# SysCV/LiDAR_snow_sim

Hardware: NVIDIA H100
Metric: augmented LiDAR points/sec (higher is better)
Workload: dtype f64

## Files before the change

include/lidar_snow_sim.h:

```cpp
#ifndef LIDAR_SNOW_SIM_H
#define LIDAR_SNOW_SIM_H

#include <stdint.h>

#ifdef __cplusplus
extern "C" {
#endif

#if defined(__GNUC__)
#define LSS_API __attribute__((visibility("default")))
#else
#define LSS_API
#endif

typedef struct lss_engine lss_engine;

typedef enum {
    LSS_OK = 0,
    LSS_ERR_INVALID_ARG = 1,
    LSS_ERR_CUDA = 2,
    LSS_ERR_NO_TABLE = 3,
    LSS_ERR_RANGE_INDEX = 4,
    LSS_ERR_NEGATIVE_INTENSITY = 5,
    LSS_ERR_OCCLUDER_OVERFLOW = 6,
    LSS_ERR_WORKSPACE = 7,
    LSS_ERR_NO_SENSOR = 8,
    LSS_ERR_TOO_FEW_GROUND = 9
} lss_status;

#define LSS_FLAG_THRESHOLD_FILTER 0x1u
#define LSS_FLAG_CAMERA_FOV 0x2u
#define LSS_FLAG_DEVICE_PREPASS 0x4u
#define LSS_FLAG_ASSUME_SORTED 0x8u

#define LSS_N_CHANNELS 64
#define LSS_POINT_STRIDE 5

LSS_API lss_status lss_create(int device, lss_engine **out);
LSS_API void lss_destroy(lss_engine *e);
LSS_API const char *lss_status_string(lss_status s);
LSS_API const char *lss_last_error(const lss_engine *e);
LSS_API int lss_version(void);

LSS_API lss_status lss_set_sensor(lss_engine *e, int n_channels, const double *h_focal_distance, const double *h_focal_slope,
                          const double *h_min_intensity, const double *h_max_intensity);

LSS_API lss_status lss_set_camera(lss_engine *e, const float *h_P2, const float *h_R0, const float *h_V2C, int img_h,
                          int img_w);

LSS_API lss_status lss_upload_particles(lss_engine *e, int n_planes, const double *h_xyr, const int64_t *h_plane_offsets,
                                double max_beam_divergence_rad, int n_azimuth_buckets, void *stream,
                                int *table_id_out);
LSS_API lss_status lss_upload_particles_device(lss_engine *e, int n_planes, const double *d_xyr,
                                       const int64_t *h_plane_offsets, double max_beam_divergence_rad,
                                       int n_azimuth_buckets, void *stream, int *table_id_out);
LSS_API lss_status lss_free_particles(lss_engine *e, int table_id);
LSS_API lss_status lss_table_info(lss_engine *e, int table_id, int64_t *n_particles, int64_t *n_entries, int64_t *bytes);

LSS_API lss_status lss_snowfall_batch(lss_engine *e, int table_id, const float *d_points, const int64_t *h_cloud_offsets,
                              int n_clouds, const int32_t *h_order, double beam_divergence_deg, const float *d_theta,
                              const double *h_thresh_poly, const double *h_plane_in, const int32_t *h_ymins_in,
                              double noise_floor, uint32_t flags, float *d_out_points,
                              int32_t *d_out_counts, double *d_out_stats, float *d_out_full, int32_t *d_out_perm,
                              int32_t *d_out_nocc, void *d_workspace, int64_t workspace_bytes, void *stream);
LSS_API int64_t lss_snowfall_workspace_bytes(int64_t n_total, int n_clouds);
LSS_API lss_status lss_snowfall_batch_host(lss_engine *e, int table_id, const float *h_points,
                                           const int64_t *h_cloud_offsets, int n_clouds, const int32_t *h_order,
                                           double beam_divergence_deg, const double *h_thresh_poly, double noise_floor,
                                           uint32_t flags, int n_chunks, float *h_out_points, int32_t *h_out_counts,
                                           double *h_out_stats);
LSS_API lss_status lss_snowfall_batch_host_submit(lss_engine *e, int table_id, const float *h_points,
                                                  const int64_t *h_cloud_offsets, int n_clouds, const int32_t *h_order,
                                                  double beam_divergence_deg, const double *h_thresh_poly,
                                                  double noise_floor, uint32_t flags, int n_chunks, float *h_out_points,
                                                  int32_t *h_out_counts, double *h_out_stats, int *ticket_out);
LSS_API lss_status lss_snowfall_batch_host_wait(lss_engine *e, int ticket);
LSS_API int lss_host_pipe_trace(lss_engine *e, float *out, int cap_chunks);
LSS_API lss_status lss_check_async(lss_engine *e, void *stream);
LSS_API int64_t lss_launch_count(const lss_engine *e);
LSS_API lss_status lss_noise_threshold_poly(lss_engine *e, const float *d_points, const int64_t *h_cloud_offsets,
                                    int n_clouds, double noise_floor, const double *h_plane_in,
                                    const int32_t *h_ymins_in, double *d_poly_out, double *d_plane_out,
                                    double *d_fit_out, int32_t *d_ymins_out, void *d_workspace,
                                    int64_t workspace_bytes, void *stream);
LSS_API int64_t lss_prepass_workspace_bytes(int64_t n_total, int n_clouds);

LSS_API lss_status lss_wet_ground_batch(lss_engine *e, const float *d_points, const int64_t *h_cloud_offsets,
                                const int32_t *d_cloud_counts, int n_clouds, double water_height, double pavement_depth,
                                double noise_floor, double power_factor, int flat_earth, double delta, int replace,
                                const double *h_plane_in, const int32_t *h_ymins_in, float *d_out_points,
                                double *d_out_intensity64, int32_t *d_out_counts, int32_t *d_out_passthrough,
                                double *d_out_plane, void *d_workspace, int64_t workspace_bytes, void *stream);
LSS_API int64_t lss_wet_ground_workspace_bytes(int64_t n_total, int n_clouds);

#define LSS_FOG_HARD 0x1u
#define LSS_FOG_SOFT 0x2u
#define LSS_FOG_GAIN 0x4u
LSS_API lss_status lss_fog_batch(lss_engine *e, const float *d_points, int n_features, const int64_t *h_cloud_offsets,
                                 int n_clouds, double alpha, double beta, double beta_0, const double *d_lut,
                                 uint32_t flags, int noise, int noise_variant, const uint64_t *h_rng_state,
                                 const double *d_ext_noise, double *d_out, uint8_t *d_out_fog_mask, int32_t *d_out_rank,
                                 double *d_out_info, void *d_workspace, int64_t workspace_bytes, void *stream);
LSS_API int64_t lss_fog_workspace_bytes(int64_t n_total, int n_clouds);
LSS_API lss_status lss_fog_batch_params(lss_engine *e, const float *d_points, int n_features,
                                        const int64_t *h_cloud_offsets, int n_clouds, const double *h_alpha,
                                        const double *h_beta, const double *h_beta_0, const int32_t *h_table_index,
                                        const double *d_luts, int n_tables, uint32_t flags, int noise, int noise_variant,
                                        const uint64_t *h_rng_state, const double *d_ext_noise, double *d_out,
                                        uint8_t *d_out_fog_mask, int32_t *d_out_rank, double *d_out_info,
                                        void *d_workspace, int64_t workspace_bytes, void *stream);
LSS_API int64_t lss_fog_batch_params_workspace_bytes(int64_t n_total, int n_clouds);

typedef struct lss_fog_table_params {
    double alpha, tau_h, r_1, r_2, D, ROH_T, ROH_R, GAMMA_T, GAMMA_R;
    double c_a, p_0, beta;
    double r_range, r_0_max, granularity;
    int32_t n, linear_xsi, shift, reserved;
} lss_fog_table_params;
LSS_API lss_status lss_fog_integral_tables(lss_engine *e, const lss_fog_table_params *h_params, int n_tables,
                                           double *d_out, void *d_workspace, int64_t workspace_bytes, void *stream);
LSS_API int64_t lss_fog_integral_tables_workspace_bytes(int n, int n_tables);

LSS_API lss_status lss_lisa_batch(lss_engine *e, const double *d_points, int n_features, int64_t n_points, double rain_rate,
                                  int mode, double alpha, double r_min, double r_max, double beam_divergence,
                                  double min_diameter, double range_accuracy, int signal_last,
                                  const double *d_draw_table, int table_len, uint64_t seed, double *d_out, void *stream);

LSS_API lss_status lss_voxelize_batch(lss_engine *e, const float *d_points, int n_features, const int64_t *h_cloud_offsets,
                                      const int32_t *d_cloud_counts, int n_clouds, const float *h_point_cloud_range,
                                      const float *h_voxel_size, int max_points_per_voxel, int max_voxels,
                                      int mask_xy_range, float *d_out_voxels, int32_t *d_out_coords,
                                      int32_t *d_out_num_points, int32_t *d_out_n_voxels, void *d_workspace,
                                      int64_t workspace_bytes, void *stream);
LSS_API int64_t lss_voxelize_workspace_bytes(int64_t n_total, int n_clouds, int max_points_per_voxel, int max_voxels);

#define LSS_DROR_CUBE 0x1u
#define LSS_DROR_WORK_STATS 0x100u
LSS_API lss_status lss_dror_batch(lss_engine *e, const float *d_points, int n_features, const int64_t *h_cloud_offsets,
                                  const int32_t *d_cloud_counts, int n_clouds, double alpha_deg, double beta, int k_min,
                                  double sr_min, uint32_t flags, uint8_t *d_out_keep ,
                                  float *d_out_points , int32_t *d_out_counts, int32_t *d_out_n_snow,
                                  void *d_workspace, int64_t workspace_bytes, void *stream);
LSS_API int64_t lss_dror_workspace_bytes(int64_t n_total, int n_clouds);

LSS_API lss_status lss_gather_push(lss_engine *e, const float *d_points, const int32_t *d_counts,
                                   const int64_t *d_cloud_offsets, int n_clouds, int64_t n_rows, int world, int rank,
                                   float *const *h_peer_points, int32_t *const *h_peer_counts, float *d_mc_points,
                                   int32_t *d_mc_counts, int n_blocks, void *stream);

LSS_API lss_status lss_dart_throwing(double occupancy_ratio, double precipitation_rate, double R_0, int distribution,
                             uint64_t *pcg_state, double *h_xyr, int64_t capacity, int64_t *n_out);
LSS_API lss_status lss_dart_throwing_planes(int n_planes, double occupancy_ratio, double precipitation_rate, double R_0,
                                    int distribution, uint64_t *pcg_states, double *h_xyr,
                                    int64_t capacity_per_plane, int64_t *h_counts, int n_threads);

LSS_API lss_status lss_sample_particles(lss_engine *e, int n_planes, double occupancy_ratio, double precipitation_rate,
                                double R_0, int distribution, uint64_t seed, int64_t n_candidates, double *d_xyr_out,
                                int64_t capacity_per_plane, int32_t *d_counts, double *d_candidates_out,
                                void *d_workspace, int64_t workspace_bytes, void *stream);
LSS_API int64_t lss_sample_particles_workspace_bytes(int n_planes, int64_t n_candidates);

LSS_API lss_status lss_set_profiling(lss_engine *e, int enable);
LSS_API lss_status lss_kernel_times(lss_engine *e, int reset, double *h_ms, int64_t *h_calls, int n);
LSS_API const char *lss_kernel_name(int kernel);
LSS_API lss_status lss_debug_azimuth(lss_engine *e, const float *d_y, const float *d_x, int64_t n, float *d_out, void *stream);
LSS_API lss_status lss_debug_range_grid(double *h_out);

#ifdef __cplusplus
}
#endif
#endif
```

lidar_snow_sim_b200/_lib.py:

```python
import ctypes
import os

_HERE = os.path.dirname(os.path.abspath(__file__))
LIB_PATH = os.path.join(_HERE, 'liblss_b200.so')

LSS_OK = 0
LSS_ERR_INVALID_ARG = 1
LSS_ERR_CUDA = 2
LSS_ERR_NO_TABLE = 3
LSS_ERR_RANGE_INDEX = 4
LSS_ERR_NEGATIVE_INTENSITY = 5
LSS_ERR_OCCLUDER_OVERFLOW = 6
LSS_ERR_WORKSPACE = 7
LSS_ERR_NO_SENSOR = 8
LSS_ERR_TOO_FEW_GROUND = 9

FLAG_THRESHOLD_FILTER = 0x1
FLAG_CAMERA_FOV = 0x2
FLAG_DEVICE_PREPASS = 0x4
FLAG_ASSUME_SORTED = 0x8
FOG_HARD, FOG_SOFT, FOG_GAIN = 0x1, 0x2, 0x4
DROR_CUBE, DROR_WORK_STATS = 0x1, 0x100



class FogTableParams(ctypes.Structure):
    _fields_ = [(f, ctypes.c_double) for f in ('alpha', 'tau_h', 'r_1', 'r_2', 'D', 'ROH_T', 'ROH_R', 'GAMMA_T',
                                                'GAMMA_R', 'c_a', 'p_0', 'beta', 'r_range', 'r_0_max', 'granularity')]
    _fields_ += [(f, ctypes.c_int32) for f in ('n', 'linear_xsi', 'shift', 'reserved')]


_EXC = {
    LSS_ERR_INVALID_ARG: ValueError,
    LSS_ERR_CUDA: RuntimeError,
    LSS_ERR_NO_TABLE: FileNotFoundError,
    LSS_ERR_RANGE_INDEX: IndexError,
    LSS_ERR_NEGATIVE_INTENSITY: AssertionError,
    LSS_ERR_OCCLUDER_OVERFLOW: RuntimeError,
    LSS_ERR_WORKSPACE: RuntimeError,
    LSS_ERR_NO_SENSOR: AssertionError,
    LSS_ERR_TOO_FEW_GROUND: TypeError,
}

_c = ctypes
_P = ctypes.c_void_p
SIGNATURES = [
    ('lss_create', _c.c_int, [_c.c_int, _c.POINTER(_P)]),
    ('lss_destroy', None, [_P]),
    ('lss_status_string', _c.c_char_p, [_c.c_int]),
    ('lss_last_error', _c.c_char_p, [_P]),
    ('lss_version', _c.c_int, []),
    ('lss_set_sensor', _c.c_int, [_P, _c.c_int, _P, _P, _P, _P]),
    ('lss_set_camera', _c.c_int, [_P, _P, _P, _P, _c.c_int, _c.c_int]),
    ('lss_upload_particles', _c.c_int, [_P, _c.c_int, _P, _P, _c.c_double, _c.c_int, _P, _c.POINTER(_c.c_int)]),
    ('lss_upload_particles_device', _c.c_int, [_P, _c.c_int, _P, _P, _c.c_double, _c.c_int, _P,
                                               _c.POINTER(_c.c_int)]),
    ('lss_free_particles', _c.c_int, [_P, _c.c_int]),
    ('lss_table_info', _c.c_int, [_P, _c.c_int, _c.POINTER(_c.c_int64), _c.POINTER(_c.c_int64),
                                  _c.POINTER(_c.c_int64)]),
    ('lss_snowfall_batch', _c.c_int, [_P, _c.c_int, _P, _P, _c.c_int, _P, _c.c_double, _P, _P, _P, _P, _c.c_double,
                                      _c.c_uint32, _P, _P, _P, _P, _P, _P, _P, _c.c_int64, _P]),
    ('lss_snowfall_workspace_bytes', _c.c_int64, [_c.c_int64, _c.c_int]),
    ('lss_host_pipe_trace', _c.c_int, [_P, _P, _c.c_int]),
    ('lss_snowfall_batch_host', _c.c_int, [_P, _c.c_int, _P, _P, _c.c_int, _P, _c.c_double, _P, _c.c_double, _c.c_uint32,
                                           _c.c_int, _P, _P, _P]),
    ('lss_snowfall_batch_host_submit', _c.c_int, [_P, _c.c_int, _P, _P, _c.c_int, _P, _c.c_double, _P, _c.c_double,
                                                  _c.c_uint32, _c.c_int, _P, _P, _P, _c.POINTER(_c.c_int)]),
    ('lss_snowfall_batch_host_wait', _c.c_int, [_P, _c.c_int]),
    ('lss_check_async', _c.c_int, [_P, _P]),
    ('lss_launch_count', _c.c_int64, [_P]),
    ('lss_debug_range_grid', _c.c_int, [_P]),
    ('lss_debug_azimuth', _c.c_int, [_P, _P, _P, _c.c_int64, _P, _P]),
    ('lss_noise_threshold_poly', _c.c_int, [_P, _P, _P, _c.c_int, _c.c_double, _P, _P, _P, _P, _P, _P, _P, _c.c_int64,
                                            _P]),
    ('lss_prepass_workspace_bytes', _c.c_int64, [_c.c_int64, _c.c_int]),
    ('lss_wet_ground_batch', _c.c_int, [_P, _P, _P, _P, _c.c_int, _c.c_double, _c.c_double, _c.c_double, _c.c_double,
                                        _c.c_int, _c.c_double, _c.c_int, _P, _P, _P, _P, _P, _P, _P, _P, _c.c_int64, _P]),
    ('lss_wet_ground_workspace_bytes', _c.c_int64, [_c.c_int64, _c.c_int]),
    ('lss_fog_batch', _c.c_int, [_P, _P, _c.c_int, _P, _c.c_int, _c.c_double, _c.c_double, _c.c_double, _P, _c.c_uint32,
                                 _c.c_int, _c.c_int, _P, _P, _P, _P, _P, _P, _P, _c.c_int64, _P]),
    ('lss_fog_workspace_bytes', _c.c_int64, [_c.c_int64, _c.c_int]),
    ('lss_fog_batch_params', _c.c_int, [_P, _P, _c.c_int, _P, _c.c_int, _P, _P, _P, _P, _P, _c.c_int, _c.c_uint32,
                                        _c.c_int, _c.c_int, _P, _P, _P, _P, _P, _P, _P, _c.c_int64, _P]),
    ('lss_fog_batch_params_workspace_bytes', _c.c_int64, [_c.c_int64, _c.c_int]),
    ('lss_fog_integral_tables', _c.c_int, [_P, _P, _c.c_int, _P, _P, _c.c_int64, _P]),
    ('lss_fog_integral_tables_workspace_bytes', _c.c_int64, [_c.c_int, _c.c_int]),
    ('lss_lisa_batch', _c.c_int, [_P, _P, _c.c_int, _c.c_int64, _c.c_double, _c.c_int, _c.c_double, _c.c_double, _c.c_double,
                                  _c.c_double, _c.c_double, _c.c_double, _c.c_int, _P, _c.c_int, _c.c_uint64, _P, _P]),
    ('lss_voxelize_batch', _c.c_int, [_P, _P, _c.c_int, _P, _P, _c.c_int, _P, _P, _c.c_int, _c.c_int, _c.c_int, _P, _P, _P,
                                      _P, _P, _c.c_int64, _P]),
    ('lss_voxelize_workspace_bytes', _c.c_int64, [_c.c_int64, _c.c_int, _c.c_int, _c.c_int]),
    ('lss_dror_batch', _c.c_int, [_P, _P, _c.c_int, _P, _P, _c.c_int, _c.c_double, _c.c_double, _c.c_int, _c.c_double,
                                  _c.c_uint32, _P, _P, _P, _P, _P, _c.c_int64, _P]),
    ('lss_dror_workspace_bytes', _c.c_int64, [_c.c_int64, _c.c_int]),
    ('lss_gather_push', _c.c_int, [_P, _P, _P, _P, _c.c_int, _c.c_int64, _c.c_int, _c.c_int, _P, _P, _P, _P, _c.c_int, _P]),
    ('lss_dart_throwing', _c.c_int, [_c.c_double, _c.c_double, _c.c_double, _c.c_int, _P, _P, _c.c_int64,
                                     _c.POINTER(_c.c_int64)]),
    ('lss_dart_throwing_planes', _c.c_int, [_c.c_int, _c.c_double, _c.c_double, _c.c_double, _c.c_int, _P, _P,
                                            _c.c_int64, _P, _c.c_int]),
    ('lss_sample_particles', _c.c_int, [_P, _c.c_int, _c.c_double, _c.c_double, _c.c_double, _c.c_int, _c.c_uint64,
                                        _c.c_int64, _P, _c.c_int64, _P, _P, _P, _c.c_int64, _P]),
    ('lss_sample_particles_workspace_bytes', _c.c_int64, [_c.c_int, _c.c_int64]),
    ('lss_set_profiling', _c.c_int, [_P, _c.c_int]),
    ('lss_kernel_times', _c.c_int, [_P, _c.c_int, _P, _P, _c.c_int]),
    ('lss_kernel_name', _c.c_char_p, [_c.c_int]),
]

_lib = None


def load():
    global _lib
    if _lib is not None:
        return _lib
    if not os.path.exists(LIB_PATH):
        raise ImportError(f'{LIB_PATH} not found: build it with `python -m lidar_snow_sim_b200.build` '
                          f'(or __graft_entry__.build()); this engine has no CPU fallback')
    lib = ctypes.CDLL(LIB_PATH)
    for name, res, args in SIGNATURES:
        fn = getattr(lib, name)
        fn.restype = res
        fn.argtypes = args
    _lib = lib
    return lib


def check(status, engine_handle=None):
    if status == LSS_OK:
        return
    lib = load()
    msg = lib.lss_status_string(status).decode()
    if engine_handle:
        detail = lib.lss_last_error(engine_handle).decode()
        if detail:
            msg = f'{msg}: {detail}'
    raise _EXC.get(status, RuntimeError)(msg)
```

lidar_snow_sim_b200/csrc/solve.cu:

```cuda
#include "beam.cuh"

namespace {

constexpr int SOLVE_TPB = 128;
constexpr int SOLVE_WARPS = SOLVE_TPB / 32;
#ifndef LSS_SOLVE_CTAS
#define LSS_SOLVE_CTAS 6
#endif
#ifndef LSS_SOLVE_ARENA
#define LSS_SOLVE_ARENA 160
#endif
constexpr int SOLVE_CTAS_PER_SM = LSS_SOLVE_CTAS;
constexpr int ARENA = LSS_SOLVE_ARENA;
constexpr int SOLVE_LCAP = 128;
static_assert(SOLVE_LCAP + 1 <= ARENA, "a beam with SOLVE_LCAP occluders must fit a round of the arena on its own");
constexpr unsigned FULL = 0xffffffffu;

struct Beam {
    double d, right, left;
    bool straddle;
};

__device__ __forceinline__ void beam_limits(float th32, double half_div, Beam &bm)
{
    const double thd = (double)th32;
    double right = thd - half_div, left = thd + half_div;
    if (right < 0) right += LSS_TWO_PI;
    if (left < 0) left += LSS_TWO_PI;
    if (right > LSS_TWO_PI) right -= LSS_TWO_PI;
    if (left > LSS_TWO_PI) left -= LSS_TWO_PI;
    bm.right = right; bm.left = left; bm.straddle = right > left;
}

__device__ __forceinline__ bool exact_hit(const ParticleRec *rp, const Beam &bm, double &rho, bool &right_hit, bool &left_hit)
{
    rho = rp->rho;
    if (!(rho < bm.d)) return false;
    const double phi = rp->phi, alpha = rp->alpha;
    bool inside = (bm.right <= phi) && (phi <= bm.left);
    if (bm.straddle) inside = inside || ((bm.right - LSS_TWO_PI <= phi) && (phi <= bm.left)) ||
                              ((bm.right <= phi) && (phi <= bm.left + LSS_TWO_PI));
    right_hit = within(bm.right - phi, alpha);
    left_hit = within(bm.left - phi, alpha);
    return inside || right_hit || left_hit;
}

struct Bucket {
    int e0, e1;
    float th_rel;
    long long pbase;
};

__device__ __forceinline__ Bucket beam_bucket(const DevArgs &a, int plane, float th32)
{
    const double thd = (double)th32;
    const double thm = thd >= LSS_TWO_PI ? thd - LSS_TWO_PI : thd;
    int bk = (int)(thm * a.inv_w);
    bk = bk < 0 ? 0 : (bk >= a.n_buckets ? a.n_buckets - 1 : bk);
    const int32_t *bs = a.bucket_start + (int64_t)plane * (a.n_buckets + 1) + bk;
    Bucket k;
    k.e0 = bs[0];
    k.e1 = bs[1];
    k.th_rel = (float)(thm - (bk + 0.5) * a.w);
    k.pbase = a.plane_off[plane];
    return k;
}

template <class F>
__device__ __forceinline__ int for_each_hit(const DevArgs &a, const Bucket &k, const Beam &bm, float d32, F &&f)
{
    int n = 0;
#pragma unroll 1
    for (int e = k.e0; e < k.e1; e++) {
        const EntryView en = lss_decode(__ldg(&a.entries[e]), a.zbase);
        if (!(en.x < d32)) break;
        if (!(fabsf(en.y - k.th_rel) <= en.z)) continue;
        const long long pi = k.pbase + en.idx;
        double rho;
        bool rh, lh;
        if (exact_hit(a.rec + pi, bm, rho, rh, lh)) { f((int)pi, rho, rh, lh); n++; }
    }
    return n;
}

constexpr int SURV_CAP = 20;

__device__ __forceinline__ double shfl_f64(double v, int src)
{
    const long long b = __double_as_longlong(v);
    const int lo = __shfl_sync(FULL, (int)(unsigned)b, src), hi = __shfl_sync(FULL, (int)(b >> 32), src);
    return __longlong_as_double(((long long)hi << 32) | (unsigned)lo);
}

#ifndef LSS_SCAN_CTAS
#define LSS_SCAN_CTAS 10
#endif
__global__ void __launch_bounds__(SNOW_TPB, LSS_SCAN_CTAS) k_scan(DevArgs a)
{
    __shared__ float s_rows[SNOW_WARPS][32 * 5];
    __shared__ int s_idx[SNOW_WARPS][32][SURV_CAP];
    __shared__ unsigned s_hit[SNOW_WARPS][32];
    const int lane = threadIdx.x & 31, wid = threadIdx.x >> 5;
    const int st = blockIdx.x * SNOW_WARPS + wid;
    if (st >= a.n_wtiles) return;
    const unsigned long long se = a.sched[st];
    const int b = (int)((se >> 32) & 0xffffu), w0 = (int)(unsigned)se;
    const int64_t beg = a.cloud_off[b];
    const int n = (int)(a.cloud_off[b + 1] - beg);
    const int i = w0 + lane;
    const bool active = i < n;
    const int nf_w = min(32, n - w0) * 5;
    float px = 0, py = 0, pz = 0, pint = 0, pch = 0;
    {
        const float *src = a.pts + (beg + w0) * 5;
#pragma unroll
        for (int q = 0; q < 5; q++) {
            const int f = q * 32 + lane;
            if (f < nf_w) s_rows[wid][f] = __ldcs(src + f);
        }
        __syncwarp();
        if (active) {
            const float *row = &s_rows[wid][5 * lane];
            px = row[0]; py = row[1]; pz = row[2]; pint = row[3]; pch = row[4];
        }
    }
    const float d32 = __fsqrt_rn(__fadd_rn(__fadd_rn(__fmul_rn(px, px), __fmul_rn(py, py)), __fmul_rn(pz, pz)));
    const int ch = channel_bin(pch);
    float out_l = pch;
    int ns = 0;
    Bucket bkt;
    bkt.e0 = bkt.e1 = 0; bkt.th_rel = 0.0f; bkt.pbase = 0;
    bool slow = false;
    float th32 = 0.0f;
    Beam bm;
    bm.d = (double)d32; bm.right = bm.left = 0.0; bm.straddle = false;
    if (active && ch < LSS_N_CHANNELS) {
        out_l = 0.0f;
        th32 = a.theta ? a.theta[beg + i] : azimuth32(py, px);
        if (th32 < 0.0f) th32 = __fadd_rn(th32, 6.2831855f);
        beam_limits(th32, a.half_div, bm);
        const int plane = a.order[b * LSS_N_CHANNELS + ch];
        if (plane >= 0 && plane < a.n_planes && th32 == th32) {
            bkt = beam_bucket(a, plane, th32);
            const int e1 = bkt.e1;
            int *pos = s_idx[wid][lane];
            bool stop = false;
#pragma unroll 1
            for (int e = bkt.e0; e < e1 && !stop; e += 4) {
                BroadEntry raw[4];
#pragma unroll
                for (int q = 0; q < 4; q++) raw[q] = __ldg(&a.entries[min(e + q, e1 - 1)]);
#pragma unroll
                for (int q = 0; q < 4; q++) {
                    if (stop || e + q >= e1) continue;
                    const EntryView en = lss_decode(raw[q], a.zbase);
                    if (!(en.x < d32)) { stop = true; continue; }
                    if (!(fabsf(en.y - bkt.th_rel) <= en.z)) continue;
                    if (ns < SURV_CAP) pos[ns] = en.idx;
                    else slow = true;
                    ns++;
                }
            }
        }
    }
    s_hit[wid][lane] = 0u;
    const int mine = slow ? 0 : ns;
    int incl = mine;
#pragma unroll
    for (int sft = 1; sft < 32; sft <<= 1) {
        const int t = __shfl_up_sync(FULL, incl, sft);
        if (lane >= sft) incl += t;
    }
    const int off = incl - mine;
    const int total = __shfl_sync(FULL, incl, 31);
    __syncwarp();
#pragma unroll 1
    for (int s0 = 0; s0 < total; s0 += 32) {
        const int s = s0 + lane;
        int j = 0;
#pragma unroll
        for (int step = 16; step; step >>= 1) {
            const int c = j + step;
            const int oc = __shfl_sync(FULL, off, c & 31);
            if (c < 32 && oc <= s) j = c;
        }
        const int r = s - __shfl_sync(FULL, off, j);
        const long long pbj = __shfl_sync(FULL, bkt.pbase, j);
        Beam bj;
        bj.d = shfl_f64(bm.d, j);
        bj.right = shfl_f64(bm.right, j);
        bj.left = shfl_f64(bm.left, j);
        bj.straddle = bj.right > bj.left;
        if (s < total) {
            double rho;
            bool rh, lh;
            if (exact_hit(a.rec + pbj + s_idx[wid][j][r], bj, rho, rh, lh)) atomicOr(&s_hit[wid][j], 1u << r);
        }
    }
    __syncwarp();
    unsigned hits = s_hit[wid][lane];
    int L = __popc(hits);
    if (slow) L = for_each_hit(a, bkt, bm, d32, [](int, double, bool, bool) {});
    {
        const bool push = L > 0;
        const unsigned pm = __ballot_sync(FULL, push);
        int lincl = push ? L : 0;
#pragma unroll
        for (int sft = 1; sft < 32; sft <<= 1) {
            const int t = __shfl_up_sync(FULL, lincl, sft);
            if (lane >= sft) lincl += t;
        }
        const int ltotal = __shfl_sync(FULL, lincl, 31);
        if (pm) {
            int hbase = 0;
            const int leader = __ffs(pm) - 1;
            if (lane == leader) hbase = atomicAdd(a.hdr + 2, ltotal);
            hbase = __shfl_sync(FULL, hbase, leader);
            if (push) {
                const int cls = LIST_CLASSES - 1 - min(LIST_CLASSES - 1, 2 * min(L, 63) + (d32 > 40.0f ? 1 : 0));
                const unsigned cm = __match_any_sync(pm, cls);
                const int cl = __ffs(cm) - 1;
                int j = 0;
                if (lane == cl) j = atomicAdd(a.hdr + LIST_CLASSES + cls, __popc(cm));
                j = __shfl_sync(cm, j, cl) + __popc(cm & ((1u << lane) - 1u));
                int *ct = a.chunk_tab + (int64_t)cls * a.chunks_per_class + j / LIST_CHUNK;
                if (j % LIST_CHUNK == 0) atomicExch(ct, atomicAdd(a.hdr, 1) + 1);
                __syncwarp(pm);
                int chunk;
                while ((chunk = *(volatile int *)ct) == 0) {}
                const int hoff = hbase + lincl - L;
                const bool fits = hoff + L <= a.hit_cap;
                {
                    SolveItem it;
                    it.key = ((unsigned long long)ch << 56) | ((unsigned long long)cls << 48) |
                             ((unsigned long long)b << 32) | (unsigned)i;
                    it.hit_off = fits ? hoff : -1;
                    it.L = L;
                    it.th32 = th32;
                    it.px = px;
                    it.py = py;
                    it.pz = pz;
                    a.items[(int64_t)(chunk - 1) * LIST_CHUNK + j % LIST_CHUNK] = it;
                }
                if (fits) {
                    int *hp = a.hit_idx + hoff;
                    if (!slow) {
                        const int *pos = s_idx[wid][lane];
#pragma unroll 1
                        for (int k = 0; hits; hits &= hits - 1) hp[k++] = (int)bkt.pbase + pos[__ffs(hits) - 1];
                    } else {
                        for_each_hit(a, bkt, bm, d32, [&](int pi, double, bool, bool) { *hp++ = pi; });
                    }
                }
            }
        }
    }
    __syncwarp();
    if (active) {
        float *row = &s_rows[wid][5 * lane];
        const float out_i = rintf(pint);
        row[3] = out_i;
        row[4] = out_l;
        if (a.nocc) a.nocc[beg + i] = 0;
        a.keep_d[beg + i] = d32;
        a.keep_i[beg + i] = out_i;
        a.keep_tag[beg + i] = (uint8_t)ch;
    }
    __syncwarp();
    {
        float *dst = a.aug + (beg + w0) * 5;
#pragma unroll
        for (int q = 0; q < 5; q++) {
            const int f = q * 32 + lane;
            if (f < nf_w) dst[f] = s_rows[wid][f];
        }
    }
}

__device__ __forceinline__ unsigned long long pack_win(int ks, int ke, int k0)
{
    return (unsigned long long)(unsigned)ks | ((unsigned long long)(unsigned)ke << 11) | ((unsigned long long)(unsigned)k0 << 22);
}

__device__ __forceinline__ void pulse_phase(double r, double &sb, double &cb)
{
    const double ctau = 299792458.0 * 1e-8, inv_ctau = 1.0 / (299792458.0 * 1e-8);
    const double bh = r * inv_ctau;
    const double bl = fma(-bh, ctau, r) * inv_ctau;
    double s, c;
    sincospi(bh, &s, &c);
    const double corr = LSS_PI * bl;
    sb = fma(corr, c, s);
    cb = fma(-corr, s, c);
}

__global__ void __launch_bounds__(SOLVE_TPB, SOLVE_CTAS_PER_SM) k_solve(DevArgs a, int *tile_cursor)
{
    __shared__ double s_arena[SOLVE_WARPS][4][ARENA];
    __shared__ unsigned long long s_piece[SOLVE_WARPS][2 * ARENA];
    __shared__ int s_piece_k[SOLVE_WARPS][2 * ARENA];
    const int lane = threadIdx.x & 31, wid = threadIdx.x >> 5;
    unsigned long long *PD = s_piece[wid];
    int *PK = s_piece_k[wid];
    double *A0 = s_arena[wid][0], *A1 = s_arena[wid][1], *A2 = s_arena[wid][2], *A3 = s_arena[wid][3];
    unsigned long long *W = reinterpret_cast<unsigned long long *>(A2);

    __shared__ int s_tile0[LIST_CLASSES + 1];
    const int *cls_cnt = a.hdr + LIST_CLASSES;
    if (wid == 0) {
        int run = 0;
        for (int c0 = 0; c0 < LIST_CLASSES; c0 += 32) {
            const int v = (cls_cnt[c0 + lane] + 31) >> 5;
            int incl = v;
#pragma unroll
            for (int sft = 1; sft < 32; sft <<= 1) {
                const int t = __shfl_up_sync(FULL, incl, sft);
                if (lane >= sft) incl += t;
            }
            s_tile0[c0 + lane] = run + incl - v;
            run += __shfl_sync(FULL, incl, 31);
        }
        if (lane == 0) s_tile0[LIST_CLASSES] = run;
    }
    __syncthreads();
    const int n_tiles = s_tile0[LIST_CLASSES];
    const double ctau = 299792458.0 * 1e-8;
    const double inv_step = (double)(LSS_M_EXT - 1) / (120 + ctau);

    for (;;) {
        int tile = 0;
        if (lane == 0) tile = atomicAdd(tile_cursor, 1);
        tile = __shfl_sync(FULL, tile, 0);
        if (tile >= n_tiles) break;
        int cls = 0;
#pragma unroll
        for (int step = LIST_CLASSES / 2; step; step >>= 1)
            if (s_tile0[cls + step] <= tile) cls += step;
        const int j = (tile - s_tile0[cls]) * 32 + lane;
        const bool active = j < cls_cnt[cls];
        SolveItem it;
        it.key = 0ull; it.hit_off = 0; it.L = 0; it.th32 = 0.0f; it.px = 0.0f; it.py = 0.0f; it.pz = 0.0f;
        if (active) {
            const int chunk = a.chunk_tab[(int64_t)cls * a.chunks_per_class + j / LIST_CHUNK];
            it = a.items[(int64_t)(chunk - 1) * LIST_CHUNK + j % LIST_CHUNK];
        }
        const int b = (int)((it.key >> 32) & 0xffffu);
        const int i = (int)(it.key & 0xffffffffu);
        const int ch = (int)(it.key >> 56);
        const int64_t beg = a.cloud_off[b];
        const float px = it.px, py = it.py, pz = it.pz;
        const float d32 = __fsqrt_rn(__fadd_rn(__fadd_rn(__fmul_rn(px, px), __fmul_rn(py, py)), __fmul_rn(pz, pz)));

        float out_x = px, out_y = py, out_z = pz, out_i = 0.0f, out_l = 0.0f;
        long long att_new_i = -1;
        int n_claim = 0;

        const int L = active ? it.L : 0;
        Beam bm;
        bm.d = (double)d32;
        beam_limits(it.th32, a.half_div, bm);

        if (L > SOLVE_LCAP) raise_status(a.status, LSS_ERR_OCCLUDER_OVERFLOW);
        const int need = (L > 0 && L <= SOLVE_LCAP) ? L + 1 : 0;

        unsigned remaining = __ballot_sync(FULL, need > 0);
        while (remaining) {
            const bool rem = (remaining >> lane) & 1u;
            const int mine = rem ? need : 0;
            int incl = mine;
#pragma unroll
            for (int s = 1; s < 32; s <<= 1) {
                const int t = __shfl_up_sync(FULL, incl, s);
                if (lane >= s) incl += t;
            }
            const bool in_round = rem && incl <= ARENA;
            remaining &= ~__ballot_sync(FULL, in_round);
            const int off = incl - mine;
            const int total = (int)__reduce_max_sync(FULL, in_round ? (unsigned)incl : 0u);
            int n_pulses = 0;
            double amax = 0.0;
            double best = 0.0;
            int kbest = 0;

#pragma unroll 1
            for (int s0 = 0; s0 < total; s0 += 32) {
                const int s = s0 + lane;
                int j = 0;
#pragma unroll
                for (int step = 16; step; step >>= 1) {
                    const int c = j + step;
                    const int oc = __shfl_sync(FULL, off, c & 31);
                    if (c < 32 && oc <= s) j = c;
                }
                const int r = s - __shfl_sync(FULL, off, j);
                const int Lj = __shfl_sync(FULL, L, j);
                const int hoj = __shfl_sync(FULL, it.hit_off, j);
                const int inr = __shfl_sync(FULL, (int)in_round, j);
                Beam bj;
                bj.d = shfl_f64(bm.d, j);
                bj.right = shfl_f64(bm.right, j);
                bj.left = shfl_f64(bm.left, j);
                bj.straddle = bj.right > bj.left;
                if (s < total && inr && r < Lj && hoj >= 0) {
                    const int pi = a.hit_idx[hoj + r];
                    const ParticleTan tn = a.tan[pi];
                    double rho;
                    bool rh, lh;
                    exact_hit(a.rec + pi, bj, rho, rh, lh);
                    A0[s] = rh ? bj.right : tn.t_right;
                    A1[s] = lh ? bj.left : tn.t_left;
                    A2[s] = rho;
                }
            }
            if (in_round && it.hit_off < 0) {
                const Bucket bkt = beam_bucket(a, a.order[b * LSS_N_CHANNELS + ch], it.th32);
                int s = off;
                for_each_hit(a, bkt, bm, d32, [&](int pi, double rho, bool rh, bool lh) {
                    A0[s] = rh ? bm.right : a.tan[pi].t_right;
                    A1[s] = lh ? bm.left : a.tan[pi].t_left;
                    A2[s] = rho;
                    s++;
                });
            }
            __syncwarp();

            if (in_round) {
#pragma unroll 1
                for (int p = 1; p < L; p++) {
                    const double rho = A2[off + p];
                    if (!(A2[off + p - 1] > rho)) continue;
                    const double a1 = A0[off + p], a2 = A1[off + p];
                    int q = p - 1;
#pragma unroll 1
                    while (q >= 0 && A2[off + q] > rho) { A0[off + q + 1] = A0[off + q]; A1[off + q + 1] = A1[off + q]; A2[off + q + 1] = A2[off + q]; q--; }
                    A0[off + q + 1] = a1; A1[off + q + 1] = a2; A2[off + q + 1] = rho;
                }

                double rb = bm.right;
                if (bm.straddle) rb = bm.right - LSS_TWO_PI;
                int nu = 0, P = 0;
                double ep_min = fmin(rb, bm.left), ep_max = fmax(rb, bm.left), claimed_total = 0.0;
#pragma unroll 1
                for (int j = 0; j < L; j++) {
                    double lo = A0[off + j];
                    const double hi = A1[off + j], rho = A2[off + j];
                    if (bm.straddle && lo > hi) lo -= LSS_TWO_PI;
                    ep_min = fmin(ep_min, fmin(lo, hi));
                    ep_max = fmax(ep_max, fmax(lo, hi));
                    if (!(lo < hi)) continue;
                    bool contained = false;
                    double cov = 0.0, nlo = lo, nhi = hi;
                    int w = 0;
#pragma unroll 1
                    for (int u = 0; u < nu; u++) {
                        const double ul = A0[off + u], uh = A1[off + u];
                        if ((ul <= lo) && (hi <= uh)) { contained = true; break; }
                        if (ul <= hi && uh >= lo) {
                            const double ov = fmin(hi, uh) - fmax(lo, ul);
                            if (ov > 0.0) cov += ov;
                            nlo = fmin(nlo, ul);
                            nhi = fmax(nhi, uh);
                        } else {
                            A0[off + w] = ul; A1[off + w] = uh; w++;
                        }
                    }
                    if (contained) continue;
                    const double claimed = (hi - lo) - cov;
                    claimed_total += claimed;
                    A0[off + w] = nlo; A1[off + w] = nhi;
                    nu = w + 1;
                    double ratio = claimed / a.div_rad;
                    ratio = ratio < 0 ? 0 : (ratio > 1 ? 1 : ratio);
                    A2[off + P] = rho;
                    A3[off + P] = ratio;
                    P++;
                }
                n_claim = P;
                double ratio_hard = ((ep_max - ep_min) - claimed_total) / a.div_rad;
                ratio_hard = ratio_hard < 0 ? 0 : (ratio_hard > 1 ? 1 : ratio_hard);

                if (P > 0) {
                    const double beta_0 = 1 * 1e-06 / LSS_PI;
                    const double i_orig = 0.9 * a.sensor->max_intensity[ch];
                    const double A = (i_orig / beta_0) * beta_0;
                    bool bad = false;
#pragma unroll 1
                    for (int j = 0; j < P; j++) {
                        const double r = A2[off + j], ratio = A3[off + j];
                        const int ks = (int)ceil(r * 10);
                        const int ke = (int)(floor((r + ctau) * 10) + 1);
                        bad |= (ke > LSS_M_EXT) || (ks < 0);
                        double sb, cb;
                        pulse_phase(r, sb, cb);
                        const double amp = (A * ratio * xsi64(r)) / (r * r);
                        amax = fmax(amax, amp);
                        A0[off + j] = amp;
                        A1[off + j] = sb;
                        A3[off + j] = cb;
                        W[off + j] = pack_win(ks, ke, (int)rint((r + ctau / 2) * inv_step));
                    }
                    {
                        const int ks = (int)ceilf(__fmul_rn(d32, 10.0f));
                        const int ke = (int)(floorf(__fmul_rn(__fadd_rn(d32, (float)ctau), 10.0f)) + 1.0f);
                        bad |= (ke > LSS_M_EXT) || (ks < 0);
                        double sb, cb;
                        pulse_phase(bm.d, sb, cb);
                        const double amp = (A * ratio_hard * xsi32(d32)) / (double)__fmul_rn(d32, d32);
                        amax = fmax(amax, amp);
                        A0[off + P] = amp;
                        A1[off + P] = sb;
                        A3[off + P] = cb;
                        W[off + P] = pack_win(ks, ke, (int)rint((bm.d + ctau / 2) * inv_step));
                    }
                    if (bad) raise_status(a.status, LSS_ERR_RANGE_INDEX);
                    else n_pulses = P + 1;
                }
            }

            int np_mine = 0;
            if (n_pulses > 0) {
                const double lb = 0.99 * amax;
                double asum = 0.0;
                int qa = 0, qb = -1, nxt = 0;
                int ks_n = (int)(W[off] & 2047u);
                int ke_a = 0;
                int k = ks_n;
                unsigned long long *pd = PD + 2 * off;
#pragma unroll 1
                for (;;) {
#pragma unroll 1
                    while (ks_n <= k) {
                        qb = nxt++;
                        asum += A0[off + qb];
                        ks_n = nxt < n_pulses ? (int)(W[off + nxt] & 2047u) : 4096;
                    }
#pragma unroll 1
                    while (qa <= qb) {
                        ke_a = (int)((W[off + qa] >> 11) & 2047u);
                        if (ke_a > k) break;
                        asum -= A0[off + qa];
                        qa++;
                    }
                    if (qa > qb) {
                        asum = 0.0;
                        if (nxt >= n_pulses) break;
                        k = ks_n;
                        continue;
                    }
                    const int pend = min(ke_a, ks_n);
                    if (asum * 1.0001 >= lb)
                        pd[np_mine++] = (unsigned long long)(unsigned)k | ((unsigned long long)(unsigned)pend << 11) |
                                        ((unsigned long long)(unsigned)(off + qa) << 22) | ((unsigned long long)(unsigned)(off + qb) << 32);
                    k = pend;
                }
            }
            int pincl = np_mine;
#pragma unroll
            for (int sft = 1; sft < 32; sft <<= 1) {
                const int t = __shfl_up_sync(FULL, pincl, sft);
                if (lane >= sft) pincl += t;
            }
            const int pex = pincl - np_mine;
            const int ptotal = __shfl_sync(FULL, pincl, 31);
            __syncwarp();
            {
                const float step = (float)((120 + ctau) / (double)(LSS_M_EXT - 1));
                const float ctau_f = (float)ctau;
#pragma unroll 1
                for (int f0 = 0; f0 < ptotal; f0 += 32) {
                    const int f = f0 + lane;
                    int j = 0;
#pragma unroll
                    for (int stp = 16; stp; stp >>= 1) {
                        const int c = j + stp;
                        const int oc = __shfl_sync(FULL, pex, c & 31);
                        if (c < 32 && oc <= f) j = c;
                    }
                    const int slot = 2 * __shfl_sync(FULL, off, j) + (f - __shfl_sync(FULL, pex, j));
                    if (f < ptotal) {
                        const unsigned long long d = PD[slot];
                        const int lo = (int)(d & 2047u), hi = (int)((d >> 11) & 2047u);
                        const int qa = (int)((d >> 22) & 1023u), qb = (int)((d >> 32) & 1023u);
                        double pbest = 0.0;
                        int pk = lo;
                        auto eval = [&](int c) {
                            const double2 t = __ldg(&a.wtab[c]);
                            double v = 0.0;
#pragma unroll 1
                            for (int q = qa; q <= qb; q++) {
                                const double sn = t.x * A3[q] - t.y * A1[q];
                                v += A0[q] * (sn * sn);
                            }
                            if (v > pbest) { pbest = v; pk = c; }
                        };
                        int kc;
                        bool all = false;
                        if (qa == qb) {
                            kc = (int)((W[qa] >> 22) & 2047u);
                        } else {
                            float zx = 0.0f, zy = 0.0f, asum = 0.0f;
#pragma unroll 1
                            for (int q = qa; q <= qb; q++) {
                                const float A = (float)A0[q], sn = (float)A1[q], cs = (float)A3[q];
                                zx += A * (cs * cs - sn * sn);
                                zy += A * (2.0f * sn * cs);
                                asum += A;
                            }
                            all = zx * zx + zy * zy < 1e-6f * asum * asum;
                            const float r0 = (atan2f(zy, zx) + 3.14159265f) * (ctau_f * 0.15915494f);
                            const float rc = 0.5f * (float)(lo + hi - 1) * step;
                            kc = (int)rintf((r0 + rintf((rc - r0) / ctau_f) * ctau_f) / step);
                        }
                        const int c_lo = all ? lo : max(lo, min(hi - 1, kc - 1));
                        const int c_hi = all ? hi - 1 : min(hi - 1, max(lo, kc + 1));
#pragma unroll 1
                        for (int c = c_lo; c <= c_hi; c++) eval(c);
                        PD[slot] = (unsigned long long)__double_as_longlong(pbest);
                        PK[slot] = pk;
                    }
                }
            }
            __syncwarp();
#pragma unroll 1
            for (int r = 0; r < np_mine; r++) {
                const double v = __longlong_as_double((long long)PD[2 * off + r]);
                if (v > best) { best = v; kbest = PK[2 * off + r]; }
            }
            __syncwarp();

            if (n_pulses > 0) {
                const double max_i = a.sensor->max_intensity[ch];
                const double min_i = a.sensor->min_intensity[ch];
                const double d_max = ((double)kbest / 10) - (ctau / 2);
                const double q1 = 1 - d_max / 120;
                double i_max = best + max_i * a.sensor->focal_slope[ch] * fabs(a.sensor->focal_offset[ch] - q1 * q1);
                i_max = i_max < min_i ? min_i : (i_max > max_i ? max_i : i_max);
                const long long new_i = (long long)i_max;
                if (fabs(d_max - bm.d) < 2 * (1.0 / 10)) {
                    out_l = 1.0f;
                    att_new_i = new_i;
                } else {
                    out_l = 2.0f;
                    const double sc = d_max / bm.d;
                    out_x = (float)((double)px * sc);
                    out_y = (float)((double)py * sc);
                    out_z = (float)((double)pz * sc);
                }
                if (new_i < 0) raise_status(a.status, LSS_ERR_NEGATIVE_INTENSITY);
                double ci = (double)new_i;
                ci = ci < min_i ? min_i : (ci > max_i ? max_i : ci);
                out_i = (float)ci;
            }
            __syncwarp();
        }

        if (active) {
            if (out_l != 0.0f) {
                const float ri = rintf(out_i);
                float *row = a.aug + (beg + i) * 5;
                row[0] = out_x; row[1] = out_y; row[2] = out_z; row[3] = ri; row[4] = out_l;
                a.keep_i[beg + i] = ri;
                a.keep_tag[beg + i] = keep_tag_of(ch, out_l);
            }
            if (a.nocc) a.nocc[beg + i] = n_claim;
        }
        {
            const bool on = att_new_i >= 0;
            const int key = b * LSS_N_CHANNELS + (ch < LSS_N_CHANNELS ? ch : 0);
            const unsigned mk = __match_any_sync(FULL, on ? key : -1);
            if (on && lane == __ffs(mk) - 1) atomicAdd(a.att_cnt + key, (unsigned)__popc(mk));
            const unsigned mb = __match_any_sync(FULL, on ? b : -1);
            const unsigned sum = __reduce_add_sync(mb, on ? (unsigned)att_new_i : 0u);
            if (on && lane == __ffs(mb) - 1) atomicAdd(&a.att_sum[b], (unsigned long long)sum);
        }
    }
}

}

namespace {
__global__ void k_debug_azimuth(const float *y, const float *x, float *out, int64_t n)
{
    const int64_t i = (int64_t)blockIdx.x * blockDim.x + threadIdx.x;
    if (i < n) out[i] = azimuth32(y[i], x[i]);
}
}

extern "C" lss_status lss_debug_azimuth(lss_engine *e, const float *d_y, const float *d_x, int64_t n, float *d_out, void *stream)
{
    if (!e || !d_y || !d_x || !d_out || n < 0) return LSS_ERR_INVALID_ARG;
    if (n == 0) return LSS_OK;
    DeviceGuard g(e->device);
    LSS_CUDA_CHECK(e, lss_launch(e, k_debug_azimuth, (unsigned)((n + 255) / 256), 256, 0, (cudaStream_t)stream, d_y, d_x,
                                 d_out, n));
    return LSS_OK;
}

cudaError_t lss_launch_scan(lss_engine *e, const DevArgs &a, cudaStream_t stream)
{
    return lss_launch(e, k_scan, (unsigned)((a.n_wtiles + SNOW_WARPS - 1) / SNOW_WARPS), SNOW_TPB, 0, stream, a);
}

cudaError_t lss_launch_solve(lss_engine *e, const DevArgs &a, int *tile_cursor, cudaStream_t stream)
{
    return lss_launch(e, k_solve, (unsigned)(e->n_sm * SOLVE_CTAS_PER_SM), SOLVE_TPB, 0, stream, a, tile_cursor);
}
```

Before: 4.300 billion.

## Prefetch next solve tile and stage particle records via cp.async

The solve kernel now claims the next tile early and loads its chunk and item in the middle of processing the current tile, so the dependent global loads overlap with compute. Occluder hit indices and particle records/tangents are gathered into shared memory with cp.async in two stages instead of per-lane scattered loads inside the exact-hit loop. Class counts are cached in shared memory. CTAs per SM drops from 6 to 5, presumably to make room for the extra registers and state. An optional clock-based phase profiler and a debug API are added, compiled out by default.

```diff
diff --git a/include/lidar_snow_sim.h b/include/lidar_snow_sim.h
--- a/include/lidar_snow_sim.h
+++ b/include/lidar_snow_sim.h
@@ -164,6 +164,8 @@
 LSS_API lss_status lss_kernel_times(lss_engine *e, int reset, double *h_ms, int64_t *h_calls, int n);
 LSS_API const char *lss_kernel_name(int kernel);
 LSS_API lss_status lss_debug_azimuth(lss_engine *e, const float *d_y, const float *d_x, int64_t n, float *d_out, void *stream);
+#define LSS_DEBUG_SOLVE_PHASE_WORDS 137
+LSS_API lss_status lss_debug_solve_phases(lss_engine *e, int reset, uint64_t *h_out, int n);
 LSS_API lss_status lss_debug_range_grid(double *h_out);
 
 #ifdef __cplusplus
diff --git a/lidar_snow_sim_b200/_lib.py b/lidar_snow_sim_b200/_lib.py
--- a/lidar_snow_sim_b200/_lib.py
+++ b/lidar_snow_sim_b200/_lib.py
@@ -71,6 +71,7 @@
     ('lss_launch_count', _c.c_int64, [_P]),
     ('lss_debug_range_grid', _c.c_int, [_P]),
     ('lss_debug_azimuth', _c.c_int, [_P, _P, _P, _c.c_int64, _P, _P]),
+    ('lss_debug_solve_phases', _c.c_int, [_P, _c.c_int, _P, _c.c_int]),
     ('lss_noise_threshold_poly', _c.c_int, [_P, _P, _P, _c.c_int, _c.c_double, _P, _P, _P, _P, _P, _P, _P, _c.c_int64,
                                             _P]),
     ('lss_prepass_workspace_bytes', _c.c_int64, [_c.c_int64, _c.c_int]),
diff --git a/lidar_snow_sim_b200/csrc/solve.cu b/lidar_snow_sim_b200/csrc/solve.cu
--- a/lidar_snow_sim_b200/csrc/solve.cu
+++ b/lidar_snow_sim_b200/csrc/solve.cu
@@ -5,7 +5,7 @@
 constexpr int SOLVE_TPB = 128;
 constexpr int SOLVE_WARPS = SOLVE_TPB / 32;
 #ifndef LSS_SOLVE_CTAS
-#define LSS_SOLVE_CTAS 6
+#define LSS_SOLVE_CTAS 5
 #endif
 #ifndef LSS_SOLVE_ARENA
 #define LSS_SOLVE_ARENA 160
@@ -294,6 +294,59 @@
     cb = fma(-corr, s, c);
 }
 
+__device__ __forceinline__ void cp_async4(void *dst, const void *src)
+{
+    asm volatile("cp.async.ca.shared.global [%0], [%1], 4;\n" ::"r"((unsigned)__cvta_generic_to_shared(dst)), "l"(src) : "memory");
+}
+__device__ __forceinline__ void cp_async8(void *dst, const void *src)
+{
+    asm volatile("cp.async.ca.shared.global [%0], [%1], 8;\n" ::"r"((unsigned)__cvta_generic_to_shared(dst)), "l"(src) : "memory");
+}
+__device__ __forceinline__ void cp_async_wait_all() { asm volatile("cp.async.wait_all;\n" ::: "memory"); }
+
+#ifdef LSS_SOLVE_PHASE_CLOCKS
+enum { PH_FETCH, PH_FILL, PH_CLAIM, PH_PULSES, PH_SWEEP, PH_EVAL, PH_STORE, PH_N };
+static_assert(PH_N + 2 + LIST_CLASSES == LSS_DEBUG_SOLVE_PHASE_WORDS, "layout of lss_debug_solve_phases");
+__device__ unsigned long long g_solve_phase[LSS_DEBUG_SOLVE_PHASE_WORDS];
+#define PHASE_INIT()                                                                                                  \
+    __shared__ unsigned long long s_ph[SOLVE_WARPS][PH_N + 1];                                                        \
+    if (lane <= PH_N) s_ph[wid][lane] = 0ull;                                                                         \
+    unsigned ph_t = (unsigned)clock64();                         \
+    unsigned ph_split = 0u
+#define PHASE(k)                                                                                                      \
+    do {                                                                                                              \
+        const unsigned ph_n = (unsigned)clock64();                                                                    \
+        if (lane == 0) s_ph[wid][k] += ph_n - ph_t;                                                                   \
+        ph_t = ph_n;                                                                                                  \
+    } while (0)
+#define PHASE_MARK() (ph_split = (unsigned)clock64() - ph_t)
+#define PHASE_SPLIT(k0, k1)                                                                                           \
+    do {                                                                                                              \
+        const unsigned ph_n = (unsigned)clock64();                                                                    \
+        const unsigned sp = __reduce_max_sync(FULL, ph_split);                                                        \
+        if (lane == 0) { s_ph[wid][k0] += sp; s_ph[wid][k1] += ph_n - ph_t - sp; }                                   \
+        ph_t = ph_n;                                                                                                  \
+        ph_split = 0u;                                                                                                \
+    } while (0)
+#define PHASE_TILE(cls, active)                                                                                       \
+    do {                                                                                                              \
+        const unsigned nb = __popc(__ballot_sync(FULL, active));                                                      \
+        if (lane == 0) { s_ph[wid][PH_N]++; atomicAdd(&g_solve_phase[PH_N + 2 + (cls)], (unsigned long long)nb); }    \
+    } while (0)
+#define PHASE_FLUSH()                                                                                                 \
+    do {                                                                                                              \
+        if (lane <= PH_N) atomicAdd(&g_solve_phase[lane], s_ph[wid][lane]);                                           \
+        if (lane == 0) atomicAdd(&g_solve_phase[PH_N + 1], 1ull);                                                     \
+    } while (0)
+#else
+#define PHASE_INIT()
+#define PHASE(k)
+#define PHASE_MARK()
+#define PHASE_SPLIT(k0, k1)
+#define PHASE_TILE(cls, active)
+#define PHASE_FLUSH()
+#endif
+
 __global__ void __launch_bounds__(SOLVE_TPB, SOLVE_CTAS_PER_SM) k_solve(DevArgs a, int *tile_cursor)
 {
     __shared__ double s_arena[SOLVE_WARPS][4][ARENA];
@@ -306,11 +359,13 @@
     unsigned long long *W = reinterpret_cast<unsigned long long *>(A2);
 
     __shared__ int s_tile0[LIST_CLASSES + 1];
-    const int *cls_cnt = a.hdr + LIST_CLASSES;
+    __shared__ int s_cnt[LIST_CLASSES];
     if (wid == 0) {
         int run = 0;
         for (int c0 = 0; c0 < LIST_CLASSES; c0 += 32) {
-            const int v = (cls_cnt[c0 + lane] + 31) >> 5;
+            const int n = a.hdr[LIST_CLASSES + c0 + lane];
+            s_cnt[c0 + lane] = n;
+            const int v = (n + 31) >> 5;
             int incl = v;
 #pragma unroll
             for (int sft = 1; sft < 32; sft <<= 1) {
@@ -326,24 +381,48 @@
     const int n_tiles = s_tile0[LIST_CLASSES];
     const double ctau = 299792458.0 * 1e-8;
     const double inv_step = (double)(LSS_M_EXT - 1) / (120 + ctau);
-
-    for (;;) {
-        int tile = 0;
-        if (lane == 0) tile = atomicAdd(tile_cursor, 1);
-        tile = __shfl_sync(FULL, tile, 0);
-        if (tile >= n_tiles) break;
-        int cls = 0;
+    PHASE_INIT();
+
+    const auto beam_of = [&](int t, int &c, int &j) {
+        c = 0;
 #pragma unroll
         for (int step = LIST_CLASSES / 2; step; step >>= 1)
-            if (s_tile0[cls + step] <= tile) cls += step;
-        const int j = (tile - s_tile0[cls]) * 32 + lane;
-        const bool active = j < cls_cnt[cls];
-        SolveItem it;
-        it.key = 0ull; it.hit_off = 0; it.L = 0; it.th32 = 0.0f; it.px = 0.0f; it.py = 0.0f; it.pz = 0.0f;
-        if (active) {
-            const int chunk = a.chunk_tab[(int64_t)cls * a.chunks_per_class + j / LIST_CHUNK];
-            it = a.items[(int64_t)(chunk - 1) * LIST_CHUNK + j % LIST_CHUNK];
-        }
+            if (s_tile0[c + step] <= t) c += step;
+        j = (t - s_tile0[c]) * 32 + lane;
+        return t < n_tiles && j < s_cnt[c];
+    };
+    const auto chunk_of = [&](int c, int j) { return a.chunk_tab[(int64_t)c * a.chunks_per_class + j / LIST_CHUNK]; };
+    const auto item_of = [&](int chunk, int j) { return a.items[(int64_t)(chunk - 1) * LIST_CHUNK + j % LIST_CHUNK]; };
+    const auto empty_item = [] {
+        SolveItem e;
+        e.key = 0ull; e.hit_off = 0; e.L = 0; e.th32 = 0.0f; e.px = 0.0f; e.py = 0.0f; e.pz = 0.0f;
+        return e;
+    };
+    int tile = 0;
+    if (lane == 0) tile = atomicAdd(tile_cursor, 1);
+    tile = __shfl_sync(FULL, tile, 0);
+    SolveItem it = empty_item();
+    {
+        int c, j;
+        if (beam_of(tile, c, j)) it = item_of(chunk_of(c, j), j);
+    }
+
+    while (tile < n_tiles) {
+        int cls, jn;
+        const bool active = beam_of(tile, cls, jn);
+        int nxt = 0;
+        if (lane == 0) nxt = atomicAdd(tile_cursor, 1);
+        int nchunk = 0;
+        bool fetched = false;
+        SolveItem nx = empty_item();
+        const auto next_chunk = [&] {
+            nxt = __shfl_sync(FULL, nxt, 0);
+            if (beam_of(nxt, cls, jn)) nchunk = chunk_of(cls, jn);
+        };
+        const auto next_item = [&] {
+            if (nchunk > 0) nx = item_of(nchunk, jn);
+            fetched = true;
+        };
         const int b = (int)((it.key >> 32) & 0xffffu);
         const int i = (int)(it.key & 0xffffffffu);
         const int ch = (int)(it.key >> 56);
@@ -362,6 +441,8 @@
 
         if (L > SOLVE_LCAP) raise_status(a.status, LSS_ERR_OCCLUDER_OVERFLOW);
         const int need = (L > 0 && L <= SOLVE_LCAP) ? L + 1 : 0;
+        PHASE_TILE(cls, active);
+        PHASE(PH_FETCH);
 
         unsigned remaining = __ballot_sync(FULL, need > 0);
         while (remaining) {
@@ -396,19 +477,44 @@
                 const int Lj = __shfl_sync(FULL, L, j);
                 const int hoj = __shfl_sync(FULL, it.hit_off, j);
                 const int inr = __shfl_sync(FULL, (int)in_round, j);
+                if (s < total) {
+                    PK[ARENA + s] = j;
+                    if (inr && r < Lj && hoj >= 0) cp_async4(&PK[s], &a.hit_idx[hoj + r]);
+                    else PK[s] = -1;
+                }
+            }
+            cp_async_wait_all();
+            __syncwarp();
+#pragma unroll 1
+            for (int s = lane; s < total; s += 32) {
+                const int pi = PK[s];
+                if (pi >= 0) {
+                    cp_async8(&A0[s], &a.rec[pi].phi);
+                    cp_async8(&A1[s], &a.rec[pi].rho);
+                    cp_async8(&A2[s], &a.rec[pi].alpha);
+                    cp_async8(&A3[s], &a.tan[pi].t_right);
+                    cp_async8(&PD[s], &a.tan[pi].t_left);
+                }
+            }
+            cp_async_wait_all();
+            __syncwarp();
+#pragma unroll 1
+            for (int s0 = 0; s0 < total; s0 += 32) {
+                const int s = s0 + lane;
+                const int j = s < total ? PK[ARENA + s] : 0;
                 Beam bj;
                 bj.d = shfl_f64(bm.d, j);
                 bj.right = shfl_f64(bm.right, j);
                 bj.left = shfl_f64(bm.left, j);
                 bj.straddle = bj.right > bj.left;
-                if (s < total && inr && r < Lj && hoj >= 0) {
-                    const int pi = a.hit_idx[hoj + r];
-                    const ParticleTan tn = a.tan[pi];
+                if (s < total && PK[s] >= 0) {
+                    ParticleRec rc;
+                    rc.phi = A0[s]; rc.rho = A1[s]; rc.alpha = A2[s];
                     double rho;
                     bool rh, lh;
-                    exact_hit(a.rec + pi, bj, rho, rh, lh);
-                    A0[s] = rh ? bj.right : tn.t_right;
-                    A1[s] = lh ? bj.left : tn.t_left;
+                    exact_hit(&rc, bj, rho, rh, lh);
+                    A0[s] = rh ? bj.right : A3[s];
+                    A1[s] = lh ? bj.left : __longlong_as_double((long long)PD[s]);
                     A2[s] = rho;
                 }
             }
@@ -423,6 +529,8 @@
                 });
             }
             __syncwarp();
+            if (!fetched) next_chunk();
+            PHASE(PH_FILL);
 
             if (in_round) {
 #pragma unroll 1
@@ -478,6 +586,7 @@
                 n_claim = P;
                 double ratio_hard = ((ep_max - ep_min) - claimed_total) / a.div_rad;
                 ratio_hard = ratio_hard < 0 ? 0 : (ratio_hard > 1 ? 1 : ratio_hard);
+                PHASE_MARK();
 
                 if (P > 0) {
                     const double beta_0 = 1 * 1e-06 / LSS_PI;
@@ -516,6 +625,8 @@
                     else n_pulses = P + 1;
                 }
             }
+            PHASE_SPLIT(PH_CLAIM, PH_PULSES);
+            if (!fetched) next_item();
 
             int np_mine = 0;
             if (n_pulses > 0) {
@@ -563,6 +674,7 @@
             const int pex = pincl - np_mine;
             const int ptotal = __shfl_sync(FULL, pincl, 31);
             __syncwarp();
+            PHASE(PH_SWEEP);
             {
                 const float step = (float)((120 + ctau) / (double)(LSS_M_EXT - 1));
                 const float ctau_f = (float)ctau;
@@ -627,6 +739,7 @@
                 if (v > best) { best = v; kbest = PK[2 * off + r]; }
             }
             __syncwarp();
+            PHASE(PH_EVAL);
 
             if (n_pulses > 0) {
                 const double max_i = a.sensor->max_intensity[ch];
@@ -652,7 +765,9 @@
                 out_i = (float)ci;
             }
             __syncwarp();
-        }
+            PHASE(PH_STORE);
+        }
+        if (!fetched) { next_chunk(); next_item(); }
 
         if (active) {
             if (out_l != 0.0f) {
@@ -673,7 +788,11 @@
             const unsigned sum = __reduce_add_sync(mb, on ? (unsigned)att_new_i : 0u);
             if (on && lane == __ffs(mb) - 1) atomicAdd(&a.att_sum[b], (unsigned long long)sum);
         }
-    }
+        PHASE(PH_STORE);
+        tile = nxt;
+        it = nx;
+    }
+    PHASE_FLUSH();
 }
 
 }
@@ -696,6 +815,24 @@
     return LSS_OK;
 }
 
+extern "C" lss_status lss_debug_solve_phases(lss_engine *e, int reset, uint64_t *h_out, int n)
+{
+    if (!e || (h_out && n < LSS_DEBUG_SOLVE_PHASE_WORDS)) return LSS_ERR_INVALID_ARG;
+#ifdef LSS_SOLVE_PHASE_CLOCKS
+    DeviceGuard g(e->device);
+    LSS_CUDA_CHECK(e, cudaDeviceSynchronize());
+    if (h_out) LSS_CUDA_CHECK(e, cudaMemcpyFromSymbol(h_out, g_solve_phase, sizeof(g_solve_phase)));
+    if (reset) {
+        static const unsigned long long zero[LSS_DEBUG_SOLVE_PHASE_WORDS] = {};
+        LSS_CUDA_CHECK(e, cudaMemcpyToSymbol(g_solve_phase, zero, sizeof(zero)));
+    }
+    return LSS_OK;
+#else
+    (void)reset;
+    return lss_fail(e, LSS_ERR_INVALID_ARG, "lss_debug_solve_phases: the library was built without -DLSS_SOLVE_PHASE_CLOCKS");
+#endif
+}
+
 cudaError_t lss_launch_scan(lss_engine *e, const DevArgs &a, cudaStream_t stream)
 {
     return lss_launch(e, k_scan, (unsigned)((a.n_wtiles + SNOW_WARPS - 1) / SNOW_WARPS), SNOW_TPB, 0, stream, a);
```

Result: faster. 4.542 billion (median of 6 runs) (+5.6%).
